# t-taniai/LocalExpStereo

Hardware: AMD Instinct MI355X
Metric: Mcost-evals/s (pixels x hypotheses / s), guided-filter cost aggregation, 1500x1000x256 vol (higher is better)
Workload: dtype i32 fixed-point box sums (exact; i64 stage-2 window sums), f32 3x3 algebra and combination

## Files before the change

__graft_entry__.py:

```python
import os
import sys

ROOT = os.path.dirname(os.path.abspath(__file__))
if ROOT not in sys.path:
    sys.path.insert(0, ROOT)


def build():
    from concurrent.futures import ThreadPoolExecutor
    from localexpstereo_amd import build as b
    with ThreadPoolExecutor(max_workers=4) as pool:
        hip = pool.submit(b.build_hip, False, True)
        sim = pool.submit(b.build_sim)
        ora = pool.submit(b.build_oracle)
        hlib = pool.submit(b.build_host_lib)
        plain = pool.submit(b.build_hip_plain)
        hip.result(); sim.result(); ora.result(); hlib.result(); plain.result()
    b.build_host()
    b.build_host_sim()
    b.build_host_selfcheck()
    import localexpstereo_amd
    from localexpstereo_amd import api
    import ctypes
    lib = ctypes.CDLL(b.HIP_SO)
    missing = [s for s in api.SYMBOLS if not hasattr(lib, s)]
    if missing:
        raise RuntimeError(f"liblocalexp_hip.so lacks symbols: {missing}")
    print("build OK:", b.HIP_SO)


def smoke():
    import numpy as np
    from localexpstereo_amd import api, synth
    from oracle import oracle as om
    H, W, D = 160, 200, 24
    imL, imR = synth.make_guide(H, W, 1234), synth.make_guide(H, W, 1235)
    volL, volR = synth.make_volume(D, H, W, 42), synth.make_volume(D, H, W, 43)
    e = api.HipCostVolumeEnergy(imL, imR, volL, volR, windR=20, eps=1e-4, th_col=0.5)
    o = om.Oracle(imL, imR, volL, volR, windR=20, eps=1e-4, th_col=0.5)
    layer = om.Layer(W, H, 20, 14)
    cells = layer.sets[5]
    rng = np.random.default_rng(0)
    planes = np.zeros((len(cells), 4), np.float32)
    planes[:, 0] = rng.uniform(-0.2, 0.2, len(cells))
    planes[:, 1] = rng.uniform(-0.2, 0.2, len(cells))
    planes[:, 2] = rng.uniform(0, D - 1, len(cells))
    frs, trs = layer.filter[cells], layer.shared[cells]
    got = e.unary_batch(frs, trs, planes, mode=0, check=True)
    ref = o.unary_batch(frs, trs, planes, mode=0, check=True)
    assert np.array_equal(np.isnan(got), np.isnan(ref)), "written region differs"
    m = ~np.isnan(ref)
    assert np.array_equal(got[m] == 1e6, ref[m] == 1e6), "invalid-label sentinels differ"
    v = m & (ref != 1e6)
    rel = np.abs(got[v] - ref[v]) / np.maximum(np.abs(ref[v]), 0.05)
    assert rel.max() <= 1e-4, f"parity failure: max rel err {rel.max()}"
    print(f"smoke OK: {len(cells)} cells, {int(v.sum())} px, max rel err {rel.max():.2e}")


if __name__ == "__main__":
    build()
    if len(sys.argv) > 1 and sys.argv[1] == "smoke":
        smoke()
```

localexpstereo_amd/build.py:

```python
import os
import shutil
import subprocess

_HERE = os.path.dirname(os.path.abspath(__file__))
ROOT = os.path.dirname(_HERE)
CSRC = os.path.join(_HERE, "csrc")
HOST = os.path.join(_HERE, "host")
HIP_SO = os.path.join(CSRC, "liblocalexp_hip.so")

HIPCC_FLAGS = ["--offload-arch=gfx950", "-O3", "-std=c++17", "-ffp-contract=off", "-fPIC", "-shared"]
HIPCC_LIBS = ["-ldl", "-lpthread"]


def _newer(target, sources):
    if not os.path.exists(target):
        return False
    t = os.path.getmtime(target)
    return all(os.path.getmtime(s) <= t for s in sources if os.path.exists(s))


def _hipcc():
    for c in (shutil.which("hipcc"), "/opt/rocm/bin/hipcc"):
        if c and os.path.exists(c):
            return c
    raise RuntimeError("hipcc not found (needed to build liblocalexp_hip.so for gfx950)")


def build_hip(force=False, verbose=False):
    srcs = [os.path.join(CSRC, f) for f in os.listdir(CSRC) if f.endswith((".hip", ".h", ".inc"))]
    srcs.append(os.path.join(ROOT, "include", "localexp_hip.h"))
    srcs += [os.path.join(HOST, f) for f in ("ResidualCut.h", "GridMaxFlow.h", "GridPushRelabel.h", "BandPool.h")]
    if not force and _newer(HIP_SO, srcs):
        return HIP_SO
    cmd = [_hipcc()] + HIPCC_FLAGS + [os.path.join(CSRC, "les_hip.hip"), "-o", HIP_SO] + HIPCC_LIBS
    if verbose:
        print(" ".join(cmd))
    subprocess.check_call(cmd, cwd=CSRC)
    return HIP_SO


PLAIN_SO = os.path.join(CSRC, "libles_plain.so")
PLAIN_FLAGS = ["-DLES_MARCH_SCAN_PLAIN", "-DLES_MARCH_STATS_PLAIN", "-DLES_SIMT_PLAIN"]


def build_hip_plain(force=False):
    srcs = [os.path.join(CSRC, f) for f in os.listdir(CSRC) if f.endswith((".hip", ".h", ".inc"))] + [os.path.join(ROOT, "include", "localexp_hip.h")]
    srcs += [os.path.join(HOST, f) for f in ("ResidualCut.h", "GridMaxFlow.h", "GridPushRelabel.h", "BandPool.h")]
    if not force and _newer(PLAIN_SO, srcs):
        return PLAIN_SO
    cmd = [_hipcc()] + HIPCC_FLAGS + PLAIN_FLAGS + [os.path.join(CSRC, "les_hip.hip"), "-o", PLAIN_SO] + HIPCC_LIBS
    subprocess.check_call(cmd, cwd=CSRC)
    return PLAIN_SO


def _build_host_demo(name, lib, force):
    exe = os.path.join(HOST, name)
    srcs = [os.path.join(HOST, f) for f in os.listdir(HOST) if f.endswith((".h", ".cpp"))] if os.path.isdir(HOST) else []
    main = os.path.join(HOST, "les_host_demo.cpp")
    if not os.path.exists(main):
        return None
    if not force and _newer(exe, srcs + [lib]):
        return exe
    libdir, libname = os.path.dirname(lib), os.path.basename(lib)[len("lib"):-len(".so")]
    cmd = ["g++", "-O2", "-std=c++17", "-fopenmp", "-ffp-contract=off", "-I", os.path.join(ROOT, "include"), main, "-o", exe,
           "-L", libdir, "-l" + libname, "-Wl,-rpath," + libdir, "-ldl"]
    subprocess.check_call(cmd, cwd=HOST)
    return exe


def build_host(force=False):
    return _build_host_demo("les_host_demo", HIP_SO, force)


def build_host_sim(force=False):
    return _build_host_demo("les_host_demo_sim", build_sim(), force)


HOST_SO = os.path.join(HOST, "liblocalexp_host.so")


def build_host_lib(force=False):
    src = os.path.join(HOST, "les_gc.cpp")
    deps = [src, os.path.join(ROOT, "include", "localexp_host.h")] + [os.path.join(HOST, f) for f in os.listdir(HOST) if f.endswith(".h")]
    if not force and _newer(HOST_SO, deps):
        return HOST_SO
    cmd = ["g++", "-O2", "-std=c++17", "-fopenmp", "-ffp-contract=off", "-fPIC", "-shared", "-I", os.path.join(ROOT, "include"), src, "-o", HOST_SO]
    subprocess.check_call(cmd, cwd=HOST)
    return HOST_SO


def build_host_selfcheck(force=False):
    src = os.path.join(ROOT, "tests", "cpp", "gc_selfcheck.cpp")
    exe = os.path.join(ROOT, "tests", "cpp", "gc_selfcheck")
    if not os.path.exists(src):
        return None
    deps = [src] + [os.path.join(HOST, f) for f in os.listdir(HOST) if f.endswith(".h")]
    if not force and _newer(exe, deps + [HIP_SO]):
        return exe
    cmd = ["g++", "-O2", "-std=c++17", "-fopenmp", "-ffp-contract=off", "-I", os.path.join(ROOT, "include"), "-I", HOST, src, "-o", exe,
           "-L", CSRC, "-llocalexp_hip", "-Wl,-rpath," + CSRC]
    subprocess.check_call(cmd, cwd=ROOT)
    return exe


def build_oracle(force=False):
# ... 12 lines not shown
```

localexpstereo_amd/csrc/les_hip_march.inc:

```
int check_rects(const les_hip_ctx* c, const les_hip_rect& f, const les_hip_rect& t)
{
    if (f.w < 0 || f.h < 0 || t.w < 0 || t.h < 0) return fail(LES_HIP_ERR_ARG, "negative rect size");
    if (f.x < 0 || f.y < 0 || f.x + f.w > c->p.W || f.y + f.h > c->p.H) return fail(LES_HIP_ERR_ARG, "filterRect outside the image");
    if (t.w > 0 && t.h > 0 && (t.x < f.x || t.y < f.y || t.x + t.w > f.x + f.w || t.y + t.h > f.y + f.h))
        return fail(LES_HIP_ERR_ARG, "targetRect not inside filterRect");
    return LES_HIP_OK;
}

int build_jobs(const les_hip_ctx* c, int n, const les_hip_rect* frs, const les_hip_rect* trs, int out_slabs,
               std::vector<les::Job>& jobs)
{
    const int TW = c->strip->TW, R = c->R;
    const long long P = (long long)c->p.H * c->p.W;
    long long strips = 0;
    for (int i = 0; i < n; i++) {
        int rc = check_rects(c, frs[i], trs[i]);
        if (rc) return rc;
        if (trs[i].w > 0 && trs[i].h > 0) strips += (trs[i].w + TW - 1) / TW;
    }
    int max_rows = 1 << 30;
    if (strips > 0 && strips < 2048) {
        long long want = (2048 + strips - 1) / strips;
        int tallest = 0;
        for (int i = 0; i < n; i++) tallest = std::max(tallest, trs[i].h);
// ... 13 lines not shown
                j.out_stride = c->p.W;
                j.plane_idx = i;
                jobs.push_back(j);
            }
    }
    std::stable_sort(jobs.begin(), jobs.end(), [](const les::Job& a, const les::Job& b) {
        if (a.tx0 != b.tx0) return a.tx0 < b.tx0;
        if (a.ty0 != b.ty0) return a.ty0 < b.ty0;
        return a.plane_idx < b.plane_idx;
    });
    return LES_HIP_OK;
}

bool build_march_jobs(les_hip_ctx* c, int n, const les_hip_rect* frs, const les_hip_rect* trs, int out_slabs,
                      std::vector<les::Job>& jobs, bool& ok, const MarchEntry*& entry)
{
    jobs.clear();
    ok = false;
    entry = nullptr;
    if (!c->march) return true;
    const int R = c->R, W = c->p.W, H = c->p.H;
    const long long P = (long long)H * W;
    ok = true;
    for (int i = 0; i < n; i++) {
        const les_hip_rect &f = frs[i], &t = trs[i];
        if (t.w <= 0 || t.h <= 0) continue;
        if ((f.x > 0 && t.x - f.x < 2 * R) || (f.x + f.w < W && (f.x + f.w) - (t.x + t.w) < 2 * R) ||
            (f.y > 0 && t.y - f.y < 2 * R) || (f.y + f.h < H && (f.y + f.h) - (t.y + t.h) < 2 * R)) ok = false;
    }
    if (!ok) {
        note_fallback(c->fallback_seen, FB_GEOMETRY, "a target rectangle lies closer than 2 x radius = %d pixels to a filterRect border that is not an image border", 2 * R);
        return true;
    }
    const int ncu = c->ncu;
    const MarchEntry* cands[2] = {c->march, find_march(c->R, 0)};
    const MarchEntry* m = c->march;
    int max_rows = 1 << 30;
    {
        double best = 1e300;
        const int row_opts[] = {1 << 30, 1024, 512, 384, 256, 192, 128, 96, 64, 48, 32};
        for (int g = 0; g < 2; g++) {
            const MarchEntry* e = cands[g];
            if (!e || (g == 1 && e == cands[0])) continue;
            if (const char* w = getenv("LES_HIP_MARCH_WIDE")) if ((atoi(w) != 0) != (g == 0)) continue;
            for (int ro : row_opts) {
                long long njobs = 0;
                int rows = 0, useful = 0;
                for (int i = 0; i < n; i++) {
                    const les_hip_rect& t = trs[i];
                    if (t.w <= 0 || t.h <= 0) continue;
                    const int ns = (t.w + e->TW - 1) / e->TW;
                    const int nr = (t.h + ro - 1) / ro, sh = (t.h + nr - 1) / nr;
                    njobs += (long long)ns * nr;
                    rows = std::max(rows, sh);
                    useful = std::max(useful, (t.w + ns - 1) / ns);
                }
                if (njobs == 0) continue;
                const long long wgs = (njobs + e->NJ - 1) / e->NJ;
                const double ticks = (double)((rows + 4 * R + e->BY - 1) / e->BY + 3);
                const double cost = (double)((wgs + ncu - 1) / ncu) * ticks * (1.0 + 1e-3 * (double)wgs / ncu) + (ro == (1 << 30) ? 0.0 : 1e-6);
                if (cost < best) { best = cost; m = e; max_rows = ro; }
            }
        }
    }
    if (const char* e = getenv("LES_HIP_MARCH_ROWS")) max_rows = std::max(1, atoi(e));
    entry = m;
    const int TW = m->TW, NJ = m->NJ;
    for (int i = 0; i < n; i++) {
        const les_hip_rect &f = frs[i], &t = trs[i];
        if (t.w <= 0 || t.h <= 0) continue;
        const int ns = (t.w + TW - 1) / TW, sw = (t.w + ns - 1) / ns;
        const int nr = (t.h + max_rows - 1) / max_rows, sh = (t.h + nr - 1) / nr;
        for (int sy = 0; sy < t.h; sy += sh)
            for (int sx = 0; sx < t.w; sx += sw) {
                les::Job j;
                j.tx0 = t.x + sx; j.ty0 = t.y + sy;
                j.tw = std::min(sw, t.w - sx); j.th = std::min(sh, t.h - sy);
                j.cx0 = f.x; j.cy0 = f.y; j.cx1 = f.x + f.w; j.cy1 = f.y + f.h;
                j.out_off = (out_slabs ? (long long)(i / out_slabs) * P : 0) + (long long)j.ty0 * W + j.tx0;
                j.out_stride = W;
                j.plane_idx = i;
                jobs.push_back(j);
            }
    }
    std::stable_sort(jobs.begin(), jobs.end(), [](const les::Job& a, const les::Job& b) {
        if (a.tx0 != b.tx0) return a.tx0 < b.tx0;
        if (a.ty0 != b.ty0) return a.ty0 < b.ty0;
        return a.plane_idx < b.plane_idx;
    });
    while (!jobs.empty() && jobs.size() % NJ) {
        les::Job pad = jobs.back();
        pad.tw = 0; pad.th = 0;
        jobs.push_back(pad);
    }
    return true;
}

int ensure_planes(les_hip_ctx* c, size_t n)
{
    if (n <= c->planes_cap) return LES_HIP_OK;
    if (c->d_planes) HIPCHECK(hipFree(c->d_planes));
    c->d_planes = nullptr; c->planes_cap = 0;
    size_t cap = std::max<size_t>(n, 1024);
    HIPCHECK(hipMalloc((void**)&c->d_planes, cap * sizeof(float4)));
    c->planes_cap = cap;
    return LES_HIP_OK;
}

struct RawPatches { const les::RawCall* calls; const long long* off; float* raw; int n, chunks; };

les::View strip_view(const les_hip_ctx* c, int mode)
{
// ... 241 lines not shown
```

localexpstereo_amd/csrc/les_march.h:

```cpp
#pragma once

#include "les_kernels.h"

#if defined(LES_MARCH_LAB)
#include "les_march_lab.h"
#else
#define LES_MARCH_ROLE_ORDER 5
#define LES_STATS_POLICY ""
#define LES_LAB_ROLE_ON(bit) true
#define LES_LAB_ABLATE(bit) false
#endif
#ifndef LES_TICK_BEGIN
#define LES_TICK_BEGIN() ((void)0)
#define LES_TICK_MARK() ((void)0)
#define LES_TICK_BARRIER() __syncthreads()
#define LES_TICK_END(role_) ((void)0)
#endif

namespace les {

constexpr int kMarchSH = 5;
constexpr int kMarchMB = 24;
constexpr int kMarchSL = 3;
constexpr int kMarchS2 = 4;
// ... 15 lines not shown
    float poff;
    float kapS;
    float upS;
    float qscale;
    float kmu;
    const long long* raw_off;
    const float* vol_t;
};
#ifndef LES_TILED_MIN_SLOPE_WIDE
#define LES_TILED_MIN_SLOPE_WIDE 0.05f
#endif
#ifndef LES_TILED_MIN_SLOPE
#define LES_TILED_MIN_SLOPE 0.125f
#endif

template <int R, int WGC, int NJ, int BY>
struct MarchCfg {
    static constexpr int KS = 2 * R + 1;
    static constexpr int RS = 3 * BY;
    static constexpr int TW = WGC - 4 * R;
    static constexpr int HWV = WGC / 64;
    static constexpr int NW = 3 * HWV * NJ;
    static constexpr int NT = 64 * NW;
    static constexpr int SEGL = 8;
    static constexpr int PADW = 16;
    static constexpr int PCOLS0 = 1 + WGC + WGC / PADW;
    static constexpr int PCOLS = PCOLS0 + ((4 - PCOLS0 % 8) + 8) % 8;
    static_assert(RS >= KS, "the ring must hold a whole window (the row that leaves it is the one written KS rows ago)");
    static_assert(RS - KS < BY, "a ring longer than the window by a block or more wastes registers: pick the smallest block height");
    static_assert(WGC % 64 == 0, "a job slot is a whole number of waves");
    static_assert(BY * (64 / SEGL) <= 64, "one wave prefixes its own tile");
    static_assert(TW > 0, "job too narrow for this radius");
    static_assert(2 * R + 1 < 64, "a window crosses at most one wave boundary");
    static_assert((long long)KS * KS * (1ll << (march_pb(R) - 1 + kMarchSL)) < (1ll << 31), "stage-1 window sums (shifted for the product with M) must fit int32");
    static_assert((long long)KS * 128 * (1ll << (march_pb(R) - 1)) < (1ll << 31), "vertical sums of Iq * pi must fit int32");
    static_assert((long long)KS * (1ll << (30 - kMarchS2)) < (1ll << 31), "the stage-2 window sums, rounded to 2^S2, must fit int32");
    __host__ __device__ static constexpr int pcol(int ci) { return 1 + ci + ci / PADW; }
};

__device__ __forceinline__ void march_prefix_scan8(int4 (&v)[8])
{
#pragma unroll
    for (int j = 1; j < 8; j++) { v[j].x += v[j - 1].x; v[j].y += v[j - 1].y; v[j].z += v[j - 1].z; v[j].w += v[j - 1].w; }
    int4 inc = v[7];
#if defined(LES_SIM) || defined(LES_MARCH_SCAN_PLAIN)
#define LES_SCAN_STEP(N) { inc.x += dpp_row_shr<N>(inc.x); inc.y += dpp_row_shr<N>(inc.y); inc.z += dpp_row_shr<N>(inc.z); inc.w += dpp_row_shr<N>(inc.w); }
    LES_SCAN_STEP(2) LES_SCAN_STEP(4) LES_SCAN_STEP(8)
#undef LES_SCAN_STEP
#else
#define LES_SCAN_ROW(N) "v_add_u32_dpp %0, %0, %0 row_shr:" #N " row_mask:0xf bank_mask:0xf bound_ctrl:1\n" \
                        "v_add_u32_dpp %1, %1, %1 row_shr:" #N " row_mask:0xf bank_mask:0xf bound_ctrl:1\n" \
                        "v_add_u32_dpp %2, %2, %2 row_shr:" #N " row_mask:0xf bank_mask:0xf bound_ctrl:1\n" \
                        "v_add_u32_dpp %3, %3, %3 row_shr:" #N " row_mask:0xf bank_mask:0xf bound_ctrl:1\n"
    asm("s_nop 1\n" LES_SCAN_ROW(2) LES_SCAN_ROW(4) LES_SCAN_ROW(8) : "+v"(inc.x), "+v"(inc.y), "+v"(inc.z), "+v"(inc.w));
#undef LES_SCAN_ROW
#endif
    const int4 off = int4{inc.x - v[7].x, inc.y - v[7].y, inc.z - v[7].z, inc.w - v[7].w};
#pragma unroll
    for (int j = 0; j < 8; j++) { v[j].x += off.x; v[j].y += off.y; v[j].z += off.z; v[j].w += off.w; }
}

template <int BY, int PCOLS>
__device__ __forceinline__ void march_prefix_tile(int4 (*T)[PCOLS], int ci0, int lane)
{
    constexpr int SEGL = 8;
    const int row = 2 * (lane >> 4) + (lane & 1), seg = (lane & 15) >> 1;
    const bool act = row < BY;
    const int c0 = ci0 + seg * SEGL;
    int4* p = &T[act ? row : 0][1 + c0 + c0 / 16];
    int4 v[SEGL];
#pragma unroll
    for (int j = 0; j < SEGL; j++) v[j] = p[j];
    march_prefix_scan8(v);
    if (act) {
#pragma unroll
        for (int j = 0; j < SEGL; j++) lds_store4(&p[j], v[j].x, v[j].y, v[j].z, v[j].w);
    }
}

template <int BY, int PCOLS>
__device__ __forceinline__ void march_prefix_pair(int4 (*TA)[PCOLS], int4 (*TB)[PCOLS], int ci0, int lane)
{
    constexpr int SEGL = 8;
    const int row = 2 * (lane >> 4) + (lane & 1), seg = (lane & 15) >> 1;
    const bool act = row < BY;
    const int c0 = ci0 + seg * SEGL;
    const int pc = 1 + c0 + c0 / 16;
    int4* pa = &TA[act ? row : 0][pc];
    int4* pb = &TB[act ? row : 0][pc];
    int4 va[SEGL], vb[SEGL];
#pragma unroll
    for (int j = 0; j < SEGL; j++) vb[j] = pb[j];
    wave_sync();
#pragma unroll
    for (int j = 0; j < SEGL; j++) va[j] = pa[j];
    LES_MARCH_SCHED_FENCE();
    march_prefix_scan8(vb);
    if (act) {
#pragma unroll
        for (int j = 0; j < SEGL; j++) lds_store4(&pb[j], vb[j].x, vb[j].y, vb[j].z, vb[j].w);
    }
    LES_MARCH_SCHED_FENCE();
    march_prefix_scan8(va);
    if (act) {
#pragma unroll
        for (int j = 0; j < SEGL; j++) lds_store4(&pa[j], va[j].x, va[j].y, va[j].z, va[j].w);
    }
// ... 44 lines not shown
    asm volatile("buffer_load_dword %0, %1, %2, %3 offen offset:32" LES_STATS_POLICY : "+v"(r.c) : "v"(voff), "s"(d), "s"(soff));
#else
    asm volatile("buffer_load_dwordx4 %0, %1, %2, %3 offen offset:32" LES_STATS_POLICY : "+v"(r.c) : "v"(voff), "s"(d), "s"(soff));
#endif
}
template <int N>
__device__ __forceinline__ void march_stats_wait(MarchStatRow& r) { asm volatile("s_waitcnt vmcnt(%3)" : "+v"(r.a), "+v"(r.b), "+v"(r.c) : "n"(N)); }
template <int N>
__device__ __forceinline__ void march_stats_wait(MarchStatRow& r, MarchStatRow& q)
{
    asm volatile("s_waitcnt vmcnt(%6)" : "+v"(r.a), "+v"(r.b), "+v"(r.c), "+v"(q.a), "+v"(q.b), "+v"(q.c) : "n"(N));
}
#endif
__device__ __forceinline__ int march_stat_m2(const MarchStatRow& r)
{
#if LES_MARCH_STAT_WORDS == 9
    return __float_as_int(r.c);
#else
    return __float_as_int(r.c.x);
#endif
}

__device__ __forceinline__ bool march_label_surely_valid(const Geom& g, float4 pl, int x0, int x1, int y0, int y1)
{
    const float ax0 = pl.x * (float)x0, ax1 = pl.x * (float)x1, by0 = pl.y * (float)y0, by1 = pl.y * (float)y1;
    const float spread = 5.0f * (fabsf(pl.x) + fabsf(pl.y));
    const float lo = (fminf(ax0, ax1) + fminf(by0, by1)) + pl.z - spread;
    const float hi = (fmaxf(ax0, ax1) + fmaxf(by0, by1)) + pl.z + spread;
    const float mag = fmaxf(fabsf(ax0), fabsf(ax1)) + fmaxf(fabsf(by0), fabsf(by1)) + fabsf(pl.z) + spread;
    const float margin = 1e-5f * mag + 1e-30f;
    return (0.0f * pl.w == 0.0f) && mag < 1e30f && (lo - margin >= g.mind) && (hi + margin <= g.maxd);
}

__device__ __forceinline__ bool march_plane_short_gather(const Geom& g, float4 pl, const Job& job, int R, int* slice_lo)
{
    *slice_lo = 0;
    const unsigned long long HW = (unsigned long long)g.H * (unsigned long long)g.W;
    const bool moderate = fabsf(pl.x) < 1e30f && fabsf(pl.y) < 1e30f && fabsf(pl.z) < 1e30f;
    if (!(moderate && g.mind == 0.0f && g.D0 == 0 && g.maxd == (float)(g.D - 1) && g.D >= 2 && HW < (1ull << 24))) return false;
    if ((unsigned long long)g.D * HW < (1ull << 30)) return true;
    const int x0 = max(job.tx0 - 2 * R, job.cx0), x1 = min(job.tx0 + job.tw + 2 * R, job.cx1) - 1;
    const int y0 = max(job.ty0 - 2 * R, job.cy0), y1 = min(job.ty0 + job.th + 2 * R, job.cy1) - 1;
    if (x1 < x0 || y1 < y0) return false;
    const float ax0 = pl.x * (float)x0, ax1 = pl.x * (float)x1, by0 = pl.y * (float)y0, by1 = pl.y * (float)y1;
    const float lo = (fminf(ax0, ax1) + fminf(by0, by1)) + pl.z, hi = (fmaxf(ax0, ax1) + fmaxf(by0, by1)) + pl.z;
    const float mag = fmaxf(fabsf(ax0), fabsf(ax1)) + fmaxf(fabsf(by0), fabsf(by1)) + fabsf(pl.z);
    const float margin = 1e-5f * mag + 1e-30f;
    if (!((lo - margin >= 0.0f) && (hi + margin < g.maxd))) return false;
    const int s0 = (int)floorf(lo - margin), s1 = (int)floorf(hi + margin) + 1;
    *slice_lo = s0;
    return s0 >= 0 && s1 < g.D && (unsigned long long)(s1 - s0 + 1) * HW < (1ull << 28);
}

template <int R, int WGC, int NJ, int BY>
__global__ void __launch_bounds__(3 * WGC * NJ)
les_march_kernel(Geom g, MarchView view, const Job* __restrict__ jobs, const float4* __restrict__ planes,
                 float* __restrict__ out, int ngroups, int check)
{
    using Cfg = MarchCfg<R, WGC, NJ, BY>;
    constexpr int KS = Cfg::KS, RS = Cfg::RS, NT = Cfg::NT, HWV = Cfg::HWV, PCOLS = Cfg::PCOLS;
    constexpr int UN = 3;

    __shared__ int4 s_T1[2][NJ][BY][PCOLS];
    __shared__ int4 s_T2[3][NJ][BY][PCOLS];
    __shared__ float s_rtab[KS + 1];

    int grp;
    {
        const int nwg = (int)gridDim.x, orig = (int)blockIdx.x;
        const int q = nwg / 8, r = nwg % 8, xcd = orig % 8;
        grp = (xcd < r ? xcd * (q + 1) : r * (q + 1) + (xcd - r) * q) + orig / 8;
    }
    if (grp >= ngroups) return;
    const int tid = (int)threadIdx.x;
    const int lane = tid & 63;
    const int wave = readfirstlane_i32(tid >> 6);
    constexpr int kRoleOf[6][3] = {{0, 1, 2}, {2, 1, 0}, {1, 2, 0}, {2, 0, 1}, {1, 0, 2}, {0, 2, 1}};
    const int slot = wave / (3 * HWV), role = kRoleOf[LES_MARCH_ROLE_ORDER][(wave % (3 * HWV)) / HWV], half = wave % HWV;
    const int ci0 = half * 64, ci = ci0 + lane;
    const Job job = jobs[grp * NJ + slot];
    int th_max = 0;
#pragma unroll
    for (int s = 0; s < NJ; s++) th_max = max(th_max, jobs[grp * NJ + s].th);
    const int nblk = (th_max + 4 * R + BY - 1) / BY;
    const int nticks = nblk + 3;
    const int Ttot = job.th > 0 ? job.th + 4 * R : 0;
    const float4 plane = planes[job.plane_idx];
    const int cy1m = max(job.cy1 - 1, job.cy0);

    if (tid <= KS) s_rtab[tid] = tid > 0 ? (float)(1.0 / (double)tid) : 0.0f;
    for (int k = tid; k < 3 * NJ * BY; k += NT) {
        if (k < 2 * NJ * BY) (&s_T1[0][0][0][0])[k * PCOLS] = int4{0, 0, 0, 0};
        (&s_T2[0][0][0][0])[k * PCOLS] = int4{0, 0, 0, 0};
    }
    __syncthreads();

    const int gx = job.tx0 - 2 * R + ci;
    const bool col_in = gx >= job.cx0 && gx < job.cx1 && job.th > 0;
    const int sx = min(max(gx, job.cx0), max(job.cx1 - 1, job.cx0));
    const uint32_t sx4 = (uint32_t)sx * 4u;
    const uint32_t rowB = (uint32_t)g.W * 4u;
    const uint32_t imgB = (uint32_t)g.H * rowB;
    const BufRsrc rs_guide = make_buf(view.ipk8, imgB);
    const int nx = window_count(gx, R, job.cx0, job.cx1);
    const int cP = min(ci + R, WGC - 1), cM = ci - R - 1;
    const int pcP = Cfg::pcol(cP);
    const int pcM = cM >= 0 ? Cfg::pcol(cM) : 0;
    const bool cross = cM >= 0 && (cP >> 6) != (cM >> 6);
    const int pcX = cross ? Cfg::pcol((cP >> 6) * 64 - 1) : 0;
    const int pcS = Cfg::pcol(ci);

    if (role == 0 && LES_LAB_ROLE_ON(1)) {
        const uint32_t HWu = (uint32_t)g.H * (uint32_t)g.W;
        const float g_ax = plane.x * (float)sx;
        const bool fronto = plane.x == 0.0f && plane.y == 0.0f;
        GatherPrep gpc = gather_prepare(g, 0.0f, plane.z, 0u, HWu, true);
        if (gpc.f1 == 0.0f) gpc.i1 = gpc.i0;
        int ringN[RS];
        uint32_t ringG[RS];
#pragma unroll
        for (int k = 0; k < RS; k++) { ringN[k] = 0; ringG[k] = 0u; }
        int Sp = 0;
        int Sc[3] = {1 << (kMarchSH - 1), 1 << (kMarchSH - 1), 1 << (kMarchSH - 1)};
        const uint32_t i0s = (uint32_t)readfirstlane_i32((int)gpc.i0), i1s = (uint32_t)readfirstlane_i32((int)gpc.i1);
        const float f1s = __int_as_float(readfirstlane_i32(__float_as_int(gpc.f1)));
        const int modes = readfirstlane_i32(gpc.mode);
        const float f0s = 1.0f - f1s;
        const bool inv_job = fronto && modes == 2 && !view.raw_off;
        int slice_lo = 0;
        const bool tame = !fronto && !view.raw_off && march_plane_short_gather(g, plane, job, R, &slice_lo);
        const uint32_t W8 = ((uint32_t)g.W + 7u) >> 3;
        const uint32_t trowB = W8 * (uint32_t)g.D * 32u;
        const int trow_lo = max(job.ty0 - 2 * R, job.cy0);
        const int trow_hi = min(job.ty0 - 2 * R + (nblk + 2) * BY, job.cy1);
        const unsigned long long tspanB = (unsigned long long)max(trow_hi - trow_lo, 1) * (unsigned long long)trowB;
        const bool tiled = tame && view.vol_t && fabsf(plane.x) >= (NJ == 1 ? LES_TILED_MIN_SLOPE_WIDE : LES_TILED_MIN_SLOPE) && tspanB < 0xfffffff0ull &&
                           (unsigned long long)W8 * (unsigned long long)g.D * 32ull < (1ull << 31);
        const float spj = !col_in ? 0.0f : (inv_job ? 0.0f : view.sp);
        const float pmj = !col_in ? __int_as_float(kMarchMagicBits) : (inv_job ? fmaf(g.th_col, view.sp, view.pmagic) : view.pmagic);
        auto march_a = [&](auto kind_tag) __attribute__((always_inline)) {
        constexpr int KIND = decltype(kind_tag)::value;
        GatherPrep gp[BY];
        float v0[BY], v1[BY];
        float f1r[BY];
        uint32_t gw[BY];
        uint32_t rowbits = 0, rowbits_nx = 0;
        int nx_rowB = 0;
        float nx_dbase = 0.0f;
        int nx_rowraw = 0;
        int nx_rowT = 0;
        const int fw = job.cx1 - job.cx0;
        const float* v0base = view.vol + (size_t)i0s;
        if constexpr (KIND == 3) v0base = view.vol + view.raw_off[job.plane_idx] - job.cx0;
        if constexpr (KIND == 4) v0base = view.vol + (size_t)slice_lo * (size_t)HWu;
        if constexpr (KIND == 5) v0base = view.vol_t + (size_t)trow_lo * (size_t)(trowB >> 2);
        const unsigned long long rest4 = (unsigned long long)(g.D - slice_lo) * (unsigned long long)imgB;
        const unsigned long long trestB = (unsigned long long)(g.H - trow_lo) * (unsigned long long)trowB;
        const uint32_t tiledB = (uint32_t)(trestB < 0xfffffffcull ? trestB : 0xfffffffcull);
        const BufRsrc rs_v0 = make_buf(v0base, KIND == 3 ? 0xfffffffcu : (KIND == 4 ? (uint32_t)(rest4 < 0xfffffffcull ? rest4 : 0xfffffffcull) : (KIND == 5 ? tiledB : imgB)));
        const uint32_t tcol = (((uint32_t)sx >> 3) * (uint32_t)g.D * 8u + ((uint32_t)sx & 7u)) * 4u;
        const int dsub = g.D0 - slice_lo;
        const BufRsrc rs_v1 = make_buf(view.vol + (size_t)i1s, imgB);
        auto prep = [&](int b) __attribute__((always_inline)) {
            const int t = b * BY + lane;
            const int gy = job.ty0 - 2 * R + t;
            const int sy = min(max(gy, job.cy0), cy1m);
            nx_rowB = (int)((uint32_t)sy * rowB);
            rowbits_nx = ballot_low(t < Ttot && gy >= job.cy0 && gy < job.cy1, BY);
            if constexpr (KIND == 3) nx_rowraw = (sy - job.cy0) * fw * 4;
            else nx_dbase = plane.y * (float)sy + plane.z;
            if constexpr (KIND == 5) nx_rowT = (int)((uint32_t)(sy - trow_lo) * trowB);
        };
        auto issue_row = [&](auto itag) __attribute__((always_inline)) {
            constexpr int i = decltype(itag)::value;
            const uint32_t ro = (uint32_t)readlane_i32(nx_rowB, i);
            if (LES_LAB_ABLATE(64)) { v0[i] = (float)lane; v1[i] = 0.0f; gw[i] = (uint32_t)lane; return; }
            if constexpr (KIND == 3) {
                v0[i] = buf_load<float>(rs_v0, sx4, (uint32_t)readlane_i32(nx_rowraw, i));
            } else if constexpr (KIND < 2) {
                v0[i] = buf_load<float>(rs_v0, sx4, ro);
                if constexpr (KIND == 1) v1[i] = buf_load<float>(rs_v1, sx4, ro);
            } else if constexpr (KIND == 4) {
                const float d = g_ax + readlane_f32(nx_dbase, i);
                const float dc = med3_f32(d, 0.0f, g.maxd);
                const float df = floorf(dc);
                f1r[i] = dc - df;
                const uint32_t e = mad_u24((int)df + dsub, (int)HWu, sx);
                v0[i] = buf_load<float>(rs_v0, e << 2, ro);
                v1[i] = buf_load<float>(rs_v0, (e << 2) + (f1r[i] > 0.0f ? imgB : 0u), ro);
            } else if constexpr (KIND == 5) {
                const float d = g_ax + readlane_f32(nx_dbase, i);
                const float dc = med3_f32(d, 0.0f, g.maxd);
                const float df = floorf(dc);
                f1r[i] = dc - df;
                const uint32_t e = (((uint32_t)(int)df + (uint32_t)g.D0) << 5) + tcol;
                const uint32_t rt = (uint32_t)readlane_i32(nx_rowT, i);
                v0[i] = buf_load<float>(rs_v0, e, rt);
                v1[i] = buf_load<float>(rs_v0, e + (f1r[i] > 0.0f ? 32u : 0u), rt);
            } else {
                const float d_base = readlane_f32(nx_dbase, i);
                const bool inside = col_in && ((rowbits_nx >> i) & 1u);
                gp[i] = gather_prepare(g, g_ax, d_base, (ro >> 2) + (uint32_t)sx, HWu, inside);
                if (gp[i].f1 == 0.0f) gp[i].i1 = gp[i].i0;
                v0[i] = view.vol[gp[i].i0];
                v1[i] = view.vol[gp[i].i1];
            }
            gw[i] = buf_load<uint32_t>(rs_guide, sx4, ro);
        };
        prep(0);
        rowbits = rowbits_nx;
        prep(0);
        static_for<BY>([&](auto itag) { issue_row(itag); });
        LES_TICK_BEGIN();
        for (int k0 = 0; k0 < nticks; k0 += UN) {
            static_for<UN>([&](auto utag) {
                constexpr int BASE = decltype(utag)::value * BY;
                const int k = k0 + decltype(utag)::value;
                if (k < nticks) {
// ... 33 lines not shown
                            Sc[2] = Sc[2] + mul24_sbyte<2>(gi, pi) + mul24_sbyte<2>(go, no);
                            lds_store4(&T[i][pcS], Sp, Sc[0] >> kMarchSH, Sc[1] >> kMarchSH, Sc[2] >> kMarchSH);
                            issue_row(itag);
                        });
                        rowbits = rowbits_nx;
                        LES_TICK_MARK();
                    }
                    {
                        int4 (*TB)[PCOLS] = s_T2[(decltype(utag)::value + UN - 2 % UN) % UN][slot];
                        const bool da = k < nblk, db = !(NJ > 1 && KIND == 2) && k >= 2 && k < nblk + 2;
                        constexpr bool kPair = KIND != 2 && KIND != 4 && KIND != 5;
                        if (kPair && da && db) march_prefix_pair<BY, PCOLS>(s_T1[k & 1][slot], TB, ci0, lane);
                        else {
                            if (da) { wave_sync(); march_prefix_tile<BY, PCOLS>(s_T1[k & 1][slot], ci0, lane); }
                            if (db) march_prefix_tile<BY, PCOLS>(TB, ci0, lane);
                        }
                    }
                    LES_TICK_BARRIER();
                }
            });
        }
        LES_TICK_END(0);
        };
        if (view.raw_off) march_a(std::integral_constant<int, 3>{});
        else if (fronto && f1s == 0.0f) march_a(std::integral_constant<int, 0>{});
        else if (fronto) march_a(std::integral_constant<int, 1>{});
        else if (tiled) march_a(std::integral_constant<int, 5>{});
        else if (tame) march_a(std::integral_constant<int, 4>{});
        else march_a(std::integral_constant<int, 2>{});
    } else if (role == 1 && LES_LAB_ROLE_ON(2)) {
        const bool s1_col = col_in && ci >= R && ci < WGC - R;
        int slice_lo_unused = 0;
        const bool general_plane = !view.raw_off && !(plane.x == 0.0f && plane.y == 0.0f) && !march_plane_short_gather(g, plane, job, R, &slice_lo_unused);
        const float kap_x = s1_col ? view.kapS * s_rtab[nx] : 0.0f;
        const float up_x = s1_col ? view.upS * s_rtab[nx] : 0.0f;
        const uint32_t sxS = (uint32_t)sx * (uint32_t)(4 * kMarchStatWords);
        const uint32_t rowS = (uint32_t)g.W * (uint32_t)(4 * kMarchStatWords);
        const MarchStatDesc ds_stats = march_stats_desc(view.mstats, (uint32_t)g.H * rowS);
        MarchStatRow st[BY];
#pragma unroll
        for (int i = 0; i < BY; i++) {
            st[i].a = st[i].b = mstat4{0.0f, 0.0f, 0.0f, 0.0f};
#if LES_MARCH_STAT_WORDS == 9
            st[i].c = 0.0f;
#else
            st[i].c = mstat4{0.0f, 0.0f, 0.0f, 0.0f};
#endif
        }
        float rny[BY];
        int nx_srow = 0;
        float nx_rny = 0.0f;
        auto prep = [&](int b) __attribute__((always_inline)) {
            const int t = b * BY + lane;
            const int gy1 = job.ty0 - 3 * R + t;
            const bool on = gy1 >= job.cy0 && gy1 < job.cy1 && t >= 2 * R && t < Ttot;
            nx_rny = on ? s_rtab[window_count(gy1, R, job.cy0, job.cy1)] : 0.0f;
            nx_srow = (int)((uint32_t)min(max(gy1, job.cy0), cy1m) * rowS);
        };
        auto issue_row = [&](auto itag) __attribute__((always_inline)) {
            constexpr int i = decltype(itag)::value;
            rny[i] = readlane_f32(nx_rny, i);
            uint32_t soff = (uint32_t)readlane_i32(nx_srow, i) & 0xfffffffcu;
            if (LES_LAB_ABLATE(4)) soff &= 0x3u;
            if (LES_LAB_ABLATE(1)) return;
            march_stats_load(st[i], ds_stats, sxS, soff);
        };
        prep(0);
        static_for<BY>([&](auto itag) { issue_row(itag); });
        LES_TICK_BEGIN();
        for (int k = 0; k < nticks; k++) {
            if (k >= 1 && k <= nblk) {
                const int b = k - 1;
                const int4 (*T1)[PCOLS] = s_T1[b & 1][slot];
                int4 (*T2)[PCOLS] = s_T2[b % 3][slot];
                constexpr int GC = 2, NS = (BY + GC - 1) / GC;
                prep(k);
                int4 pp[2][GC], pm[2][GC], px[2][GC];
                auto lds_stage = [&](auto stag) __attribute__((always_inline)) {
                    constexpr int S = decltype(stag)::value;
#pragma unroll
                    for (int j = 0; j < GC; j++)
                        if (S * GC + j < BY) {
                            if (LES_LAB_ABLATE(2)) { pp[S & 1][j] = int4{lane, k, 2, 3}; pm[S & 1][j] = int4{3, 2, k, lane}; px[S & 1][j] = int4{0, 0, 0, 0}; }
                            else { pp[S & 1][j] = T1[S * GC + j][pcP]; pm[S & 1][j] = T1[S * GC + j][pcM]; px[S & 1][j] = T1[S * GC + j][pcX]; }
                        }
                };
                lds_stage(std::integral_constant<int, 0>{});
                static_for<NS>([&](auto gtag) {
                    constexpr int S = decltype(gtag)::value, CB = S & 1;
                    constexpr int LO = S * GC;
                    constexpr int N = (BY - LO) < GC ? (BY - LO) : GC;
                    if constexpr (S + 1 < NS) lds_stage(std::integral_constant<int, S + 1>{});
                    LES_MARCH_SCHED_FENCE();
                    static_assert(GC == 2, "vmcnt bookkeeping below is written for stages of two rows");
                    if constexpr (N == 2) march_stats_wait<3 * (BY - 2)>(st[LO], st[LO + 1]);
                    else march_stats_wait<3 * (BY - 1)>(st[LO]);
                    static_for<N>([&](auto jtag) {
                        constexpr int j = decltype(jtag)::value;
                        constexpr int i = LO + j;
                        const int s = pp[CB][j].x - pm[CB][j].x + px[CB][j].x;
                        const mstat4 q0 = st[i].a, q1 = st[i].b;
                        const int M0 = __float_as_int(q1.z), M1 = __float_as_int(q1.w), M2 = march_stat_m2(st[i]);
                        const long long s8 = (long long)(s << kMarchSL);
                        const float d0 = (float)((pp[CB][j].y - pm[CB][j].y) + px[CB][j].y + (int)(((long long)M0 * s8 + (1ll << 31)) >> 32));
                        const float d1 = (float)((pp[CB][j].z - pm[CB][j].z) + px[CB][j].z + (int)(((long long)M1 * s8 + (1ll << 31)) >> 32));
                        const float d2 = (float)((pp[CB][j].w - pm[CB][j].w) + px[CB][j].w + (int)(((long long)M2 * s8 + (1ll << 31)) >> 32));
                        const float ka = kap_x * rny[i];
                        const float a0 = fmaf(q0.z, d2, fmaf(q0.y, d1, q0.x * d0)) * ka;
                        const float a1 = fmaf(q1.x, d2, fmaf(q0.w, d1, q0.y * d0)) * ka;
                        const float a2 = fmaf(q1.y, d2, fmaf(q1.x, d1, q0.z * d0)) * ka;
                        const float mp = (float)s * (up_x * rny[i]);
#if LES_MARCH_STAT_WORDS == 9
                        const float bb = fmaf(view.kmu, fmaf(a2, (float)M2, fmaf(a1, (float)M1, a0 * (float)M0)), mp);
#else
                        const float bb = fmaf(-a2, st[i].c.w, fmaf(-a1, st[i].c.z, fmaf(-a0, st[i].c.y, mp)));
#endif
                        lds_store4(&T2[i][pcS], cvt_rpi_i32(a0), cvt_rpi_i32(a1), cvt_rpi_i32(a2), cvt_rpi_i32(bb));
                    });
                    LES_MARCH_SCHED_FENCE();
                    static_for<N>([&](auto jtag) { issue_row(std::integral_constant<int, LO + decltype(jtag)::value>{}); });
                });
                LES_TICK_MARK();
            }
            if (NJ > 1 && general_plane && k >= 2 && k < nblk + 2) march_prefix_tile<BY, PCOLS>(s_T2[(k - 2) % 3][slot], ci0, lane);
            LES_TICK_BARRIER();
        }
        LES_TICK_END(1);
    } else if (role == 2 && LES_LAB_ROLE_ON(4)) {
        const bool out_col = ci >= 2 * R && ci < 2 * R + job.tw && job.th > 0;
        const uint32_t oc4 = (uint32_t)max(ci - 2 * R, 0) * 4u;
        const float vl_xa = (float)gx * plane.x, vl_c = 1.0f * plane.z, vl_zv = 0.0f * plane.w, vl_a5 = plane.x * 5, vl_b5 = plane.y * 5;
        const float c_lane = view.qscale * s_rtab[nx];
        int ring2[4][RS];
#pragma unroll
        for (int k = 0; k < RS; k++) ring2[0][k] = ring2[1][k] = ring2[2][k] = ring2[3][k] = 0;
        long long S2[4] = {1ll << (kMarchS2 - 1), 1ll << (kMarchS2 - 1), 1ll << (kMarchS2 - 1), 1ll << (kMarchS2 - 1)};
        uint32_t gq[BY];
        float rny2[BY];
        uint32_t okbits = 0;
        int nx_grow = 0;
        float nx_rny = 0.0f;
        const BufRsrc rs_out = make_buf(out + job.out_off, 0xfffffffcu);
        const uint32_t ostrideB = (uint32_t)job.out_stride * 4u;
        auto prep = [&](int b) __attribute__((always_inline)) {
            const int t = b * BY + lane;
            const int gy2 = job.ty0 - 4 * R + t;
            nx_rny = s_rtab[window_count(gy2, R, job.cy0, job.cy1)];
            nx_grow = (int)((uint32_t)min(max(gy2, job.cy0), cy1m) * rowB);
            okbits = ballot_low(t >= 4 * R && t < Ttot, BY);
        };
        auto issue_row = [&](auto itag) __attribute__((always_inline)) {
            constexpr int i = decltype(itag)::value;
            rny2[i] = readlane_f32(nx_rny, i);
            if (LES_LAB_ABLATE(128)) { gq[i] = (uint32_t)lane; return; }
            gq[i] = buf_load<uint32_t>(rs_guide, sx4, (uint32_t)readlane_i32(nx_grow, i));
        };
        auto march_d = [&](auto check_tag) __attribute__((always_inline)) {
        constexpr bool CHECK = decltype(check_tag)::value != 0;
        LES_TICK_BEGIN();
        for (int k0 = 0; k0 < nticks; k0 += UN) {
            static_for<UN>([&](auto utag) {
                constexpr int U = decltype(utag)::value;
                constexpr int BASE = ((U + UN - 3 % UN) % UN) * BY;
                const int k = k0 + U;
                if (k < nticks) {
                    if (k >= 3) {
                        const int b = k - 3;
                        const int4 (*T2)[PCOLS] = s_T2[(U + UN - 3 % UN) % UN][slot];
                        constexpr int GD = 1, NS = (BY + GD - 1) / GD;
                        int4 pp[2][GD], pm[2][GD], px[2][GD];
                        auto lds_stage = [&](auto stag) __attribute__((always_inline)) {
                            constexpr int S = decltype(stag)::value;
#pragma unroll
                            for (int j = 0; j < GD; j++)
                                if (S * GD + j < BY) {
                                    if (LES_LAB_ABLATE(16)) { pp[S & 1][j] = int4{lane, b, 2, 3}; pm[S & 1][j] = int4{3, 2, b, lane}; px[S & 1][j] = int4{0, 0, 0, 0}; }
                                    else { pp[S & 1][j] = T2[S * GD + j][pcP]; pm[S & 1][j] = T2[S * GD + j][pcM]; px[S & 1][j] = T2[S * GD + j][pcX]; }
                                }
                        };
                        lds_stage(std::integral_constant<int, 0>{});
                        static_for<NS>([&](auto gtag) {
                            constexpr int S = decltype(gtag)::value, CB = S & 1;
                            constexpr int LO = S * GD;
                            constexpr int N = (BY - LO) < GD ? (BY - LO) : GD;
                            if constexpr (S + 1 < NS) lds_stage(std::integral_constant<int, S + 1>{});
                            LES_MARCH_SCHED_FENCE();
                            static_for<N>([&](auto jtag) {
                                constexpr int j = decltype(jtag)::value;
                                constexpr int i = LO + j;
                                constexpr int SLOT = BASE + i, OLD = (SLOT + RS - KS) % RS;
                                const int h0 = pp[CB][j].x - pm[CB][j].x + px[CB][j].x, h1 = pp[CB][j].y - pm[CB][j].y + px[CB][j].y;
                                const int h2 = pp[CB][j].z - pm[CB][j].z + px[CB][j].z, h3 = pp[CB][j].w - pm[CB][j].w + px[CB][j].w;
                                const int o0 = ring2[0][OLD], o1 = ring2[1][OLD], o2 = ring2[2][OLD], o3 = ring2[3][OLD];
                                ring2[0][SLOT] = h0; ring2[1][SLOT] = h1; ring2[2][SLOT] = h2; ring2[3][SLOT] = h3;
                                acc64_add_i32(S2[0], h0 - o0); acc64_add_i32(S2[1], h1 - o1); acc64_add_i32(S2[2], h2 - o2); acc64_add_i32(S2[3], h3 - o3);
                                if (out_col && ((okbits >> i) & 1u)) {
                                    const int t = b * BY + i;
                                    const uint32_t gi = gq[i];
                                    const float f0 = (float)(int)(S2[0] >> kMarchS2), f1 = (float)(int)(S2[1] >> kMarchS2), f2 = (float)(int)(S2[2] >> kMarchS2), f3 = (float)(int)(S2[3] >> kMarchS2);
                                    const float acc = fmaf(f2, cvt_f32_sbyte<2>(gi), fmaf(f1, cvt_f32_sbyte<1>(gi), fmaf(f0, cvt_f32_sbyte<0>(gi), f3 * 255.0f)));
                                    float q = fmaf(acc * c_lane, rny2[i], view.poff);
                                    if constexpr (CHECK) {
                                        const int gy2 = job.ty0 + t - 4 * R;
                                        const float ds = ((vl_xa + (float)gy2 * plane.y) + vl_c) + vl_zv;
                                        const float dp = ds + vl_a5, dm = ds - vl_a5;
                                        const float d1 = dp + vl_b5, d2 = dp - vl_b5, d3 = dm + vl_b5, d4 = dm - vl_b5;
                                        const float mn = fmin3(fmin3(ds, d1, d2), d3, d4), mx = fmax3(fmax3(ds, d1, d2), d3, d4);
                                        if (!(mn >= g.mind && mx <= g.maxd)) q = LES_COST_INVALID;
                                    }
                                    if (!(LES_LAB_ABLATE(128) && q != 12345.0f))
                                    buf_store<float>(rs_out, oc4, (uint32_t)(t - 4 * R) * ostrideB, q);
                                }
                            });
                            LES_MARCH_SCHED_FENCE();
                        });
                    }
                    if (k >= 2 && k <= nblk + 1) {
                        prep(k - 2);
                        static_for<BY>([&](auto itag) { issue_row(itag); });
                    }
                    LES_TICK_BARRIER();
                }
            });
        }
        LES_TICK_END(2);
        };
        const bool surely_valid = march_label_surely_valid(g, plane, job.tx0, job.tx0 + max(job.tw, 1) - 1, job.ty0, job.ty0 + max(job.th, 1) - 1);
        if (check && !surely_valid) march_d(std::integral_constant<int, 1>{});
        else march_d(std::integral_constant<int, 0>{});
    }
}

__global__ void les_march_stats_kernel(const double* __restrict__ hs, const uint32_t* __restrict__ ipk, uint32_t* __restrict__ ipk8,
                                       float* __restrict__ mstats, unsigned* __restrict__ inv_diag_max, int H, int W, int R, double eps)
{
    int x = (int)(blockIdx.x * blockDim.x + threadIdx.x), y = (int)blockIdx.y;
    if (x >= W) return;
    size_t P = (size_t)H * W;
    double s[9] = {0, 0, 0, 0, 0, 0, 0, 0, 0};
    for (int dy = -R; dy <= R; dy++) {
        int yy = y + dy;
        if (yy < 0 || yy >= H) continue;
        for (int k = 0; k < 9; k++) s[k] += hs[k * P + (size_t)yy * W + x];
    }
    double N = (double)(window_count(x, R, 0, W) * window_count(y, R, 0, H));
    double m0 = s[0] / N, m1 = s[1] / N, m2 = s[2] / N;
    double rr = s[3] / N - m0 * m0 + eps, rg = s[4] / N - m0 * m1, rb = s[5] / N - m0 * m2;
    double gg = s[6] / N - m1 * m1 + eps, gb = s[7] / N - m1 * m2, bb = s[8] / N - m2 * m2 + eps;
    double irr = gg * bb - gb * gb, irg = gb * rb - rg * bb, irb = rg * gb - gg * rb;
    double igg = rr * bb - rb * rb, igb = rb * rg - rr * gb, ibb = rr * gg - rg * rg;
    double det = irr * rr + irg * rg + irb * rb;
    irr /= det; irg /= det; irb /= det; igg /= det; igb /= det; ibb /= det;
    size_t px = (size_t)y * W + x;
    const double fs = (double)(1ll << kMarchMB);
    const double c0 = m0 * 255.0 - 128.0, c1 = m1 * 255.0 - 128.0, c2 = m2 * 255.0 - 128.0;
    const int M0 = (int)fmin(fmax(rint(-c0 * fs), -2147483648.0), 2147483647.0);
    const int M1 = (int)fmin(fmax(rint(-c1 * fs), -2147483648.0), 2147483647.0);
    const int M2 = (int)fmin(fmax(rint(-c2 * fs), -2147483648.0), 2147483647.0);
    float* o = mstats + px * kMarchStatWords;
    o[0] = (float)irr; o[1] = (float)irg; o[2] = (float)irb; o[3] = (float)igg;
    o[4] = (float)igb; o[5] = (float)ibb; o[6] = __int_as_float(M0); o[7] = __int_as_float(M1);
    o[8] = __int_as_float(M2);
    if (kMarchStatWords == 12) { o[9] = (float)(c0 / 255.0); o[10] = (float)(c1 / 255.0); o[11] = (float)(c2 / 255.0); }
    const uint32_t v = ipk[px];
// ... 42 lines not shown
```

Baseline: 171,600.

## Skip march halo rows above clipped image top and tighten DPP scan

The march kernel now starts its row sweep later when the job's window halo begins above the clip boundary cy0. Rows there contribute nothing, so it skips up to 2R leading rows and shifts the stage offsets (ry0, tC, tD) to match. The host-side tile planner now uses the same row count when picking a config, and the first DPP scan step reads v[7] directly instead of modifying in place. A separate build without the skip (LES_MARCH_SKIP0) is added for comparison. The risk is off-by-one errors in the stage offsets at image boundaries.

```diff
diff --git a/__graft_entry__.py b/__graft_entry__.py
--- a/__graft_entry__.py
+++ b/__graft_entry__.py
@@ -9,13 +9,14 @@
 def build():
     from concurrent.futures import ThreadPoolExecutor
     from localexpstereo_amd import build as b
-    with ThreadPoolExecutor(max_workers=4) as pool:
+    with ThreadPoolExecutor(max_workers=6) as pool:
         hip = pool.submit(b.build_hip, False, True)
         sim = pool.submit(b.build_sim)
         ora = pool.submit(b.build_oracle)
         hlib = pool.submit(b.build_host_lib)
         plain = pool.submit(b.build_hip_plain)
-        hip.result(); sim.result(); ora.result(); hlib.result(); plain.result()
+        skip0 = pool.submit(b.build_hip_skip0)
+        hip.result(); sim.result(); ora.result(); hlib.result(); plain.result(); skip0.result()
     b.build_host()
     b.build_host_sim()
     b.build_host_selfcheck()
diff --git a/localexpstereo_amd/build.py b/localexpstereo_amd/build.py
--- a/localexpstereo_amd/build.py
+++ b/localexpstereo_amd/build.py
@@ -51,6 +51,20 @@
     cmd = [_hipcc()] + HIPCC_FLAGS + PLAIN_FLAGS + [os.path.join(CSRC, "les_hip.hip"), "-o", PLAIN_SO] + HIPCC_LIBS
     subprocess.check_call(cmd, cwd=CSRC)
     return PLAIN_SO
+
+
+SKIP0_SO = os.path.join(CSRC, "libles_skip0.so")
+SKIP0_FLAGS = ["-DLES_MARCH_SKIP0"]
+
+
+def build_hip_skip0(force=False):
+    srcs = [os.path.join(CSRC, f) for f in os.listdir(CSRC) if f.endswith((".hip", ".h", ".inc"))] + [os.path.join(ROOT, "include", "localexp_hip.h")]
+    srcs += [os.path.join(HOST, f) for f in ("ResidualCut.h", "GridMaxFlow.h", "GridPushRelabel.h", "BandPool.h")]
+    if not force and _newer(SKIP0_SO, srcs):
+        return SKIP0_SO
+    cmd = [_hipcc()] + HIPCC_FLAGS + SKIP0_FLAGS + [os.path.join(CSRC, "les_hip.hip"), "-o", SKIP0_SO] + HIPCC_LIBS
+    subprocess.check_call(cmd, cwd=CSRC)
+    return SKIP0_SO
 
 
 def _build_host_demo(name, lib, force):
diff --git a/localexpstereo_amd/csrc/les_hip_march.inc b/localexpstereo_amd/csrc/les_hip_march.inc
--- a/localexpstereo_amd/csrc/les_hip_march.inc
+++ b/localexpstereo_amd/csrc/les_hip_march.inc
@@ -89,12 +89,12 @@
                     const int ns = (t.w + e->TW - 1) / e->TW;
                     const int nr = (t.h + ro - 1) / ro, sh = (t.h + nr - 1) / nr;
                     njobs += (long long)ns * nr;
-                    rows = std::max(rows, sh);
+                    for (int sy = 0; sy < t.h; sy += sh) rows = std::max(rows, les::march_rows(R, t.y + sy, std::min(sh, t.h - sy), frs[i].y));
                     useful = std::max(useful, (t.w + ns - 1) / ns);
                 }
                 if (njobs == 0) continue;
                 const long long wgs = (njobs + e->NJ - 1) / e->NJ;
-                const double ticks = (double)((rows + 4 * R + e->BY - 1) / e->BY + 3);
+                const double ticks = (double)((rows + e->BY - 1) / e->BY + 3);
                 const double cost = (double)((wgs + ncu - 1) / ncu) * ticks * (1.0 + 1e-3 * (double)wgs / ncu) + (ro == (1 << 30) ? 0.0 : 1e-6);
                 if (cost < best) { best = cost; m = e; max_rows = ro; }
             }
diff --git a/localexpstereo_amd/csrc/les_march.h b/localexpstereo_amd/csrc/les_march.h
--- a/localexpstereo_amd/csrc/les_march.h
+++ b/localexpstereo_amd/csrc/les_march.h
@@ -91,7 +91,13 @@
                         "v_add_u32_dpp %1, %1, %1 row_shr:" #N " row_mask:0xf bank_mask:0xf bound_ctrl:1\n" \
                         "v_add_u32_dpp %2, %2, %2 row_shr:" #N " row_mask:0xf bank_mask:0xf bound_ctrl:1\n" \
                         "v_add_u32_dpp %3, %3, %3 row_shr:" #N " row_mask:0xf bank_mask:0xf bound_ctrl:1\n"
-    asm("s_nop 1\n" LES_SCAN_ROW(2) LES_SCAN_ROW(4) LES_SCAN_ROW(8) : "+v"(inc.x), "+v"(inc.y), "+v"(inc.z), "+v"(inc.w));
+    asm("s_nop 1\n"
+        "v_add_u32_dpp %0, %4, %4 row_shr:2 row_mask:0xf bank_mask:0xf bound_ctrl:1\n"
+        "v_add_u32_dpp %1, %5, %5 row_shr:2 row_mask:0xf bank_mask:0xf bound_ctrl:1\n"
+        "v_add_u32_dpp %2, %6, %6 row_shr:2 row_mask:0xf bank_mask:0xf bound_ctrl:1\n"
+        "v_add_u32_dpp %3, %7, %7 row_shr:2 row_mask:0xf bank_mask:0xf bound_ctrl:1\n"
+        LES_SCAN_ROW(4) LES_SCAN_ROW(8)
+        : "=&v"(inc.x), "=&v"(inc.y), "=&v"(inc.z), "=&v"(inc.w) : "v"(v[7].x), "v"(v[7].y), "v"(v[7].z), "v"(v[7].w));
 #undef LES_SCAN_ROW
 #endif
     const int4 off = int4{inc.x - v[7].x, inc.y - v[7].y, inc.z - v[7].z, inc.w - v[7].w};
@@ -242,6 +248,18 @@
     return s0 >= 0 && s1 < g.D && (unsigned long long)(s1 - s0 + 1) * HW < (1ull << 28);
 }
 
+__host__ __device__ inline int march_row_skip(int R, int ty0, int th, int cy0)
+{
+#if defined(LES_MARCH_SKIP0)
+    (void)R; (void)ty0; (void)th; (void)cy0;
+    return 0;
+#else
+    const int above = cy0 - (ty0 - 2 * R);
+    return th > 0 ? (above < 0 ? 0 : (above > 2 * R ? 2 * R : above)) : 0;
+#endif
+}
+__host__ __device__ inline int march_rows(int R, int ty0, int th, int cy0) { return th > 0 ? th + 4 * R - march_row_skip(R, ty0, th, cy0) : 0; }
+
 template <int R, int WGC, int NJ, int BY>
 __global__ void __launch_bounds__(3 * WGC * NJ)
 les_march_kernel(Geom g, MarchView view, const Job* __restrict__ jobs, const float4* __restrict__ planes,
@@ -269,12 +287,15 @@
     const int slot = wave / (3 * HWV), role = kRoleOf[LES_MARCH_ROLE_ORDER][(wave % (3 * HWV)) / HWV], half = wave % HWV;
     const int ci0 = half * 64, ci = ci0 + lane;
     const Job job = jobs[grp * NJ + slot];
-    int th_max = 0;
-#pragma unroll
-    for (int s = 0; s < NJ; s++) th_max = max(th_max, jobs[grp * NJ + s].th);
-    const int nblk = (th_max + 4 * R + BY - 1) / BY;
+    int rows_max = 0;
+#pragma unroll
+    for (int s = 0; s < NJ; s++) { const Job& js = jobs[grp * NJ + s]; rows_max = max(rows_max, march_rows(R, js.ty0, js.th, js.cy0)); }
+    const int nblk = (rows_max + BY - 1) / BY;
     const int nticks = nblk + 3;
-    const int Ttot = job.th > 0 ? job.th + 4 * R : 0;
+    const int skip = march_row_skip(R, job.ty0, job.th, job.cy0);
+    const int ry0 = job.ty0 - 2 * R + skip;
+    const int tC = 2 * R - skip, tD = 4 * R - skip;
+    const int Ttot = march_rows(R, job.ty0, job.th, job.cy0);
     const float4 plane = planes[job.plane_idx];
     const int cy1m = max(job.cy1 - 1, job.cy0);
 
@@ -321,8 +342,8 @@
         const bool tame = !fronto && !view.raw_off && march_plane_short_gather(g, plane, job, R, &slice_lo);
         const uint32_t W8 = ((uint32_t)g.W + 7u) >> 3;
         const uint32_t trowB = W8 * (uint32_t)g.D * 32u;
-        const int trow_lo = max(job.ty0 - 2 * R, job.cy0);
-        const int trow_hi = min(job.ty0 - 2 * R + (nblk + 2) * BY, job.cy1);
+        const int trow_lo = max(ry0, job.cy0);
+        const int trow_hi = min(ry0 + (nblk + 2) * BY, job.cy1);
         const unsigned long long tspanB = (unsigned long long)max(trow_hi - trow_lo, 1) * (unsigned long long)trowB;
         const bool tiled = tame && view.vol_t && fabsf(plane.x) >= (NJ == 1 ? LES_TILED_MIN_SLOPE_WIDE : LES_TILED_MIN_SLOPE) && tspanB < 0xfffffff0ull &&
                            (unsigned long long)W8 * (unsigned long long)g.D * 32ull < (1ull << 31);
@@ -353,7 +374,7 @@
         const BufRsrc rs_v1 = make_buf(view.vol + (size_t)i1s, imgB);
         auto prep = [&](int b) __attribute__((always_inline)) {
             const int t = b * BY + lane;
-            const int gy = job.ty0 - 2 * R + t;
+            const int gy = ry0 + t;
             const int sy = min(max(gy, job.cy0), cy1m);
             nx_rowB = (int)((uint32_t)sy * rowB);
             rowbits_nx = ballot_low(t < Ttot && gy >= job.cy0 && gy < job.cy1, BY);
@@ -493,8 +514,8 @@
         float nx_rny = 0.0f;
         auto prep = [&](int b) __attribute__((always_inline)) {
             const int t = b * BY + lane;
-            const int gy1 = job.ty0 - 3 * R + t;
-            const bool on = gy1 >= job.cy0 && gy1 < job.cy1 && t >= 2 * R && t < Ttot;
+            const int gy1 = ry0 - R + t;
+            const bool on = gy1 >= job.cy0 && gy1 < job.cy1 && t >= tC && t < Ttot;
             nx_rny = on ? s_rtab[window_count(gy1, R, job.cy0, job.cy1)] : 0.0f;
             nx_srow = (int)((uint32_t)min(max(gy1, job.cy0), cy1m) * rowS);
         };
@@ -585,10 +606,10 @@
         const uint32_t ostrideB = (uint32_t)job.out_stride * 4u;
         auto prep = [&](int b) __attribute__((always_inline)) {
             const int t = b * BY + lane;
-            const int gy2 = job.ty0 - 4 * R + t;
+            const int gy2 = ry0 - 2 * R + t;
             nx_rny = s_rtab[window_count(gy2, R, job.cy0, job.cy1)];
             nx_grow = (int)((uint32_t)min(max(gy2, job.cy0), cy1m) * rowB);
-            okbits = ballot_low(t >= 4 * R && t < Ttot, BY);
+            okbits = ballot_low(t >= tD && t < Ttot, BY);
         };
         auto issue_row = [&](auto itag) __attribute__((always_inline)) {
             constexpr int i = decltype(itag)::value;
@@ -642,7 +663,7 @@
                                     const float acc = fmaf(f2, cvt_f32_sbyte<2>(gi), fmaf(f1, cvt_f32_sbyte<1>(gi), fmaf(f0, cvt_f32_sbyte<0>(gi), f3 * 255.0f)));
                                     float q = fmaf(acc * c_lane, rny2[i], view.poff);
                                     if constexpr (CHECK) {
-                                        const int gy2 = job.ty0 + t - 4 * R;
+                                        const int gy2 = ry0 - 2 * R + t;
                                         const float ds = ((vl_xa + (float)gy2 * plane.y) + vl_c) + vl_zv;
                                         const float dp = ds + vl_a5, dm = ds - vl_a5;
                                         const float d1 = dp + vl_b5, d2 = dp - vl_b5, d3 = dm + vl_b5, d4 = dm - vl_b5;
@@ -650,7 +671,7 @@
                                         if (!(mn >= g.mind && mx <= g.maxd)) q = LES_COST_INVALID;
                                     }
                                     if (!(LES_LAB_ABLATE(128) && q != 12345.0f))
-                                    buf_store<float>(rs_out, oc4, (uint32_t)(t - 4 * R) * ostrideB, q);
+                                    buf_store<float>(rs_out, oc4, (uint32_t)(t - tD) * ostrideB, q);
                                 }
                             });
                             LES_MARCH_SCHED_FENCE();
```

Result: no change. 170,700 (-0.5%).
